# DanielPS555/Radix-sort-Merge-Sort-CUDA---Lab-y-practicos-GPGPU-2023

Hardware: AMD Instinct MI355X
Metric: Mkeys/s sorting uint32, n=2^28, 1 GPU (+ merge-sort at 2/4/8) (higher is better)
Workload: dtype u32; 1 GPU; LSD radix sort (8-bit digits, onesweep), n=2^28 uint32 u32, device-resident (BASELINE config 3); n_per_gpu=268435456, algo=radix, key=u32, dist=u32, parallelism=single GPU

## Files before the change

### include/labsort.h

```cpp
#ifndef LABSORT_H
#define LABSORT_H

#include <stddef.h>
#include <stdint.h>

#ifdef __cplusplus
extern "C" {
#endif

#define LABSORT_OK 0
#define LABSORT_ERR_ARG 1
#define LABSORT_ERR_HIP 2
#define LABSORT_ERR_DEVICE 3
#define LABSORT_ERR_PEER 4

#define LABSORT_ALGO_RADIX 0
#define LABSORT_ALGO_MERGE 1
#define LABSORT_ALGO_RADIX1 2
#define LABSORT_ALGO_AUTO 3
#define LABSORT_AUTO_MERGE_MAX_KEYS (1u << 16)
#define LABSORT_AUTO_PAIRS_MERGE_MAX_KEYS (1u << 18)

#define LABSORT_KEY_U32 0
#define LABSORT_KEY_I32 1
// ... 19 lines not shown
#define LABSORT_K_PARTITION 4
#define LABSORT_K_GSWEEP 5
#define LABSORT_K_GCOPY 6
#define LABSORT_K_COPY 7
#define LABSORT_K_MERGE4 8
#define LABSORT_K_SEGSORT 9
#define LABSORT_K_TOPK 10
#define LABSORT_K_COUNT 11

const char *labsort_version(void);
const char *labsort_error_string(int status);
int labsort_last_hip_error(void);
const char *labsort_hip_error_string(int hip_error);
size_t labsort_max_keys(int algo);
size_t labsort_tile_keys(void);
size_t labsort_merge_tile_keys(void);

size_t labsort_workspace_bytes(size_t n, int algo);
int labsort_sort_device(const void *d_in, void *d_out, size_t n, int key_type, int algo, void *d_workspace,
                        size_t workspace_bytes, void *stream);
int labsort_sort_host(void *h_keys, size_t n, int key_type, int algo);
int labsort_workspace_status(const void *d_workspace, size_t n, int algo, void *stream);
int labsort_radix_path(const void *d_workspace, size_t n, void *stream);
int labsort_pairs_workspace_status(const void *d_workspace, size_t n, int algo, void *stream);

#define LABSORT_XFER_AUTO 0
#define LABSORT_XFER_RCCL 1
#define LABSORT_XFER_PEER 2
#define LABSORT_MULTI_MAX_RANKS 8
#define LABSORT_MULTI_PHASES 9
#define LABSORT_MULTI_COLLECTIVES 3
int labsort_sort_host_multi(void *h_keys, size_t n, int key_type, int ngpus);
int labsort_sort_host_ranks(void *h_keys, size_t n, int key_type, int nranks, const int *devices, int transport);
int labsort_multi_timing(double *phase_ms, int nphases, size_t *max_sent_bytes);
int labsort_multi_collectives(double *arrive, double *leave, int nranks, int ncoll);
int labsort_multi_last_hip_error(void);
int labsort_multi_range_counts(size_t *counts, int nranks);
const char *labsort_multi_error_detail(void);
int labsort_multi_plan(const uint32_t *const *h_shards, const size_t *m, int nranks, int key_type, size_t *h_cuts);

#define LABSORT_COMM_ID_BYTES 128
#define LABSORT_DIST_MAX_RANKS 16
typedef struct labsort_comm *labsort_comm_t;
typedef struct {
    void *ctx;
    int (*allgather)(void *ctx, const void *h_in, void *h_out, size_t bytes);
// ... 84 lines not shown
```

### radix-sort-merge-sort-cuda---lab-y-practicos-gpgpu-2023_amd/__init__.py

```python
from __future__ import annotations

import ctypes
import os

import numpy as np

HERE = os.path.dirname(os.path.abspath(__file__))
LIB_PATH = os.environ.get("LABSORT_LIBRARY") or os.path.join(HERE, "liblabsort.so")

OK, ERR_ARG, ERR_HIP, ERR_DEVICE, ERR_PEER = 0, 1, 2, 3, 4
ALGO = {"radix": 0, "merge": 1, "radix1": 2, "auto": 3}
KEY = {"u32": 0, "i32": 1, "f32": 2, "bf16": 3, "f16": 4}
DIST = {"u32": 0, "u31": 1, "mod100": 2, "mod1000": 3, "sorted": 4, "reversed": 5, "const": 6, "lowbits": 7}
KCLASS = {"histogram": 0, "onesweep": 1, "tile_sort": 2, "merge": 3, "partition": 4, "gsweep": 5, "gcopy": 6,
          "copy": 7, "merge4": 8, "segsort": 9, "topk": 10}
TOPK_SORT_DIV = 4

C_SYMBOLS = [
    "labsort_version", "labsort_error_string", "labsort_last_hip_error", "labsort_hip_error_string",
    "labsort_max_keys", "labsort_tile_keys", "labsort_merge_tile_keys", "labsort_workspace_bytes",
    "labsort_sort_device", "labsort_sort_host", "labsort_wave_tile_sort", "labsort_tile_sort",
    "labsort_merge_parts", "labsort_merge_pass", "labsort_merge", "labsort_histogram", "labsort_fill",
    "labsort_count_descents", "labsort_timing_enable", "labsort_timing_read", "labsort_upper_bound", "sort",
    "labsort_merge_runs_workspace_bytes", "labsort_merge_runs",
    "labsort_pair_tile_keys", "labsort_pairs_workspace_bytes", "labsort_sort_pairs_device",
    "labsort_workspace_status", "labsort_pairs_workspace_status", "labsort_radix_path",
    "labsort_sort_host_multi", "labsort_sort_host_ranks", "labsort_multi_timing", "labsort_multi_last_hip_error",
    "labsort_multi_plan", "labsort_multi_error_detail", "labsort_multi_range_counts",
    "labsort_comm_unique_id", "labsort_comm_init_rccl", "labsort_comm_init_host", "labsort_comm_destroy",
    "labsort_dist_sort", "labsort_dist_timing", "labsort_dist_last_hip_error",
    "labsort_multi_collectives", "labsort_dist_collectives", "labsort_copy",
    "labsort_comm_set_timeout", "labsort_test_fault",
    "labsort_segment_tile_keys", "labsort_segment_pair_tile_keys", "labsort_segment_class_edges",
    "labsort_segments_workspace_bytes", "labsort_sort_segments_device", "labsort_sort_segments_pairs_device",
    "labsort_segments_workspace_status",
    "labsort_topk_workspace_bytes", "labsort_topk_device", "labsort_topk_workspace_status",
    "labsort_sort_rows_workspace_bytes", "labsort_sort_rows_device", "labsort_sort_rows_workspace_status",
    "labsort_sort16_chunk_keys", "labsort_sort16_workspace_bytes", "labsort_sort16_device",
    "labsort_sort16_workspace_status",
    "labsort_key_order_bits", "labsort_key_from_order_bits",
]
XFER = {"auto": 0, "rccl": 1, "peer": 2}
MULTI_PHASES = ["h2d", "local_sort", "plan", "exchange", "merge", "d2h", "total", "plan_work", "plan_wait"]
COLLECTIVES = ["samples", "counts", "grow"]
CXX_SYMBOLS = ["_Z11order_arrayPii", "_Z16order_with_trustPii"]


class LabsortError(RuntimeError):

# ... 55 lines not shown
    L.labsort_max_keys.argtypes = [i]
    L.labsort_tile_keys.restype = sz
    L.labsort_merge_tile_keys.restype = sz
    L.labsort_merge_parts.restype = sz
    L.labsort_merge_parts.argtypes = [sz]
    L.labsort_workspace_bytes.argtypes = [sz, i]
    L.labsort_sort_device.argtypes = [p, p, sz, i, i, p, sz, p]
    L.labsort_sort_host.argtypes = [p, sz, i, i]
    L.labsort_wave_tile_sort.argtypes = [p, sz, i, p]
    L.labsort_tile_sort.argtypes = [p, p, sz, i, p]
    L.labsort_merge_pass.argtypes = [p, p, sz, sz, i, p, p]
    L.labsort_merge.argtypes = [p, sz, p, sz, p, sz, sz, i, p, p]
    L.labsort_merge_runs_workspace_bytes.restype = sz
    L.labsort_merge_runs_workspace_bytes.argtypes = [sz]
    L.labsort_merge_runs.argtypes = [p, p, ctypes.POINTER(sz), i, i, p, sz, p]
    L.labsort_pair_tile_keys.restype = sz
    L.labsort_pair_tile_keys.argtypes = []
    L.labsort_pairs_workspace_bytes.restype = sz
    L.labsort_pairs_workspace_bytes.argtypes = [sz, i]
    L.labsort_sort_pairs_device.argtypes = [p, p, p, p, sz, i, i, p, sz, p]
    L.labsort_workspace_status.argtypes = [p, sz, i, p]
    if hasattr(L, "labsort_radix_path"):
        L.labsort_radix_path.argtypes = [p, sz, p]
    L.labsort_sort_host_multi.argtypes = [p, sz, i, i]
    L.labsort_sort_host_ranks.argtypes = [p, sz, i, i, p, i]
    L.labsort_multi_timing.argtypes = [ctypes.POINTER(ctypes.c_double), i, ctypes.POINTER(sz)]
    L.labsort_multi_plan.argtypes = [ctypes.POINTER(p), ctypes.POINTER(sz), i, i, ctypes.POINTER(sz)]
    L.labsort_multi_range_counts.argtypes = [ctypes.POINTER(sz), i]
    L.labsort_multi_error_detail.restype = ctypes.c_char_p
    L.labsort_multi_error_detail.argtypes = []
    L.labsort_comm_unique_id.argtypes = [p]
    L.labsort_comm_init_rccl.argtypes = [ctypes.POINTER(p), p, i, i]
    L.labsort_comm_init_host.argtypes = [ctypes.POINTER(p), i, i, ctypes.POINTER(HostColl)]
    L.labsort_comm_destroy.argtypes = [p]
    L.labsort_comm_set_timeout.argtypes = [p, ctypes.c_double]
    L.labsort_test_fault.argtypes = [ctypes.c_char_p, i]
    L.labsort_dist_sort.argtypes = [p, p, sz, i, p, ctypes.POINTER(p), ctypes.POINTER(sz), ctypes.POINTER(sz)]
    L.labsort_dist_timing.argtypes = [p, ctypes.POINTER(ctypes.c_double), i, ctypes.POINTER(sz)]
    L.labsort_dist_last_hip_error.argtypes = [p]
    L.labsort_multi_collectives.argtypes = [ctypes.POINTER(ctypes.c_double), ctypes.POINTER(ctypes.c_double), i, i]
    L.labsort_dist_collectives.argtypes = [p, ctypes.POINTER(ctypes.c_double), ctypes.POINTER(ctypes.c_double), i]
    L.labsort_copy.argtypes = [p, p, sz, p]
    L.labsort_pairs_workspace_status.argtypes = [p, sz, i, p]
    L.labsort_segment_tile_keys.restype = sz
    L.labsort_segment_tile_keys.argtypes = []
    L.labsort_segment_pair_tile_keys.restype = sz
# ... 284 lines not shown

def sort_device(d_in, d_out, n: int, key: str = "u32", algo: str = "radix", workspace=None,
                workspace_bytes_: int | None = None, stream=None) -> None:
    workspace, wsb, own = _workspace(workspace, lambda: workspace_bytes(n, algo))
    if workspace_bytes_ is not None:
        wsb = workspace_bytes_
    _check(lib.labsort_sort_device(_ptr(d_in), _ptr(d_out), n, KEY[key], ALGO[algo], _ptr(workspace), wsb,
                                   _stream(stream)), "sort_device")
    if own:
        workspace_status(workspace, n, algo, stream)


def workspace_status(workspace, n: int, algo: str = "radix", stream=None) -> None:
    _check(lib.labsort_workspace_status(_ptr(workspace), n, ALGO[algo], _stream(stream)), "sort_device (status)")


def radix_path(workspace, n: int, stream=None) -> int:
    r = int(lib.labsort_radix_path(_ptr(workspace), n, _stream(stream)))
    if r < 0:
        _check(-r, "radix_path")
    return r


def pairs_workspace_status(workspace, n: int, algo: str = "radix", stream=None) -> None:
    _check(lib.labsort_pairs_workspace_status(_ptr(workspace), n, ALGO[algo], _stream(stream)),
           "sort_pairs_device (status)")


def wave_tile_sort(d_keys, n: int, key: str = "u32", stream=None) -> None:
    _check(lib.labsort_wave_tile_sort(_ptr(d_keys), n, KEY[key], _stream(stream)), "wave_tile_sort")


def tile_sort(d_in, d_out, n: int, key: str = "u32", stream=None) -> None:
    _check(lib.labsort_tile_sort(_ptr(d_in), _ptr(d_out), n, KEY[key], _stream(stream)), "tile_sort")


def merge_pass(d_in, d_out, n: int, run: int, d_part, key: str = "u32", stream=None) -> None:
    _check(lib.labsort_merge_pass(_ptr(d_in), _ptr(d_out), n, run, KEY[key], _ptr(d_part), _stream(stream)),
           "merge_pass")


def merge(d_a, la: int, d_b, lb: int, d_out, d0: int, d1: int, d_part, key: str = "u32", stream=None) -> None:
    _check(lib.labsort_merge(_ptr(d_a) if la else 0, la, _ptr(d_b) if lb else 0, lb, _ptr(d_out), d0, d1,
                             KEY[key], _ptr(d_part), _stream(stream)), "merge")


# ... 224 lines not shown
```

### radix-sort-merge-sort-cuda---lab-y-practicos-gpgpu-2023_amd/csrc/api.hip

```cpp
#include <hip/hip_runtime.h>

#include <algorithm>
#include <cstdio>
#include <cstdlib>
#include <cstring>
#include <mutex>
#include <vector>

#include "host.h"
#include "segsort.h"

using namespace labsort;

namespace {

thread_local int g_last_hip = 0;

struct TimedLaunch {
    int cls;
    hipEvent_t a, b;
};
std::mutex g_timing_mu;
bool g_timing_on = false;
std::vector<TimedLaunch> g_pending;
// ... 92 lines not shown
    if (LABSORT_MERGE4)
        for (size_t r = (merge_levels(n, merge_tile(pairs)) % 2 ? 2 : 1) * merge_tile(pairs); r < n; r *= 4)
            bw = std::max(bw, merge4_bnd_words(n, r));
    L.off_bnd = c.take(bw * 4);
    for (int i = 0; i < 2; ++i) L.off_samp[i] = c.take(bw ? merge4_samp_words(n) * 4 : 0);
    L.total = c.o;
    return L;
}

bool use_gather(size_t n) {
    const char *e = std::getenv("LABSORT_RADIX_IMPL");
    if (e && !std::strcmp(e, "gather")) return true;
    if (n < GS_MIN_N || n >= GS_MAX_N) return false;
    return !(e && !std::strcmp(e, "onesweep"));
}

uint32_t hybrid_gate(size_t n) {
    const char *e = std::getenv("LABSORT_RADIX_HYBRID");
    if (e && !std::strcmp(e, "0")) return 0u;
    if (e && !std::strcmp(e, "2")) return HY_MAX_BUCKET;
    return n >= HY_MIN_N && n <= HY_MAX_N ? HY_FAST_GROUP : 0u;
}

bool small_path(size_t n, int algo) { return algo != LABSORT_ALGO_RADIX1 && n <= (size_t)TS_TILE; }

int sort_radix8(const uint32_t *ki, const uint32_t *vi, uint32_t *ko, uint32_t *vo, size_t n, uint32_t flip, char *ws,
                hipStream_t s) {
    const RadixLayout L = radix_layout(n, 8, OSP_TILE);
    Bufs b, vb;
    b.p[SEL_IN] = const_cast<uint32_t *>(ki);
    b.p[SEL_OUT] = ko;
    b.p[SEL_TMP] = reinterpret_cast<uint32_t *>(ws + L.off_tmp);
    vb.p[SEL_IN] = const_cast<uint32_t *>(vi);
    vb.p[SEL_OUT] = vo;
    vb.p[SEL_TMP] = vi ? reinterpret_cast<uint32_t *>(ws + align_up(L.total, 256)) : nullptr;
    uint32_t *hist = reinterpret_cast<uint32_t *>(ws + L.off_hist);
    uint32_t *counters = reinterpret_cast<uint32_t *>(ws + L.off_counter);
    uint32_t *err = reinterpret_cast<uint32_t *>(ws + L.off_err);
    uint32_t *lookback = reinterpret_cast<uint32_t *>(ws + L.off_lookback);
    Plan *plan = reinterpret_cast<Plan *>(ws + L.off_plan);
    HIP_TRY(launch_zero(ws, L.off_lookback, s));
    uint32_t *hps = reinterpret_cast<uint32_t *>(ws + L.off_hps);
    uint32_t *joint = reinterpret_cast<uint32_t *>(ws + L.off_joint);
    SegPlan *sps = reinterpret_cast<SegPlan *>(ws + L.off_segplan);
    const uint32_t hy_limit = vi ? 0u : hybrid_gate(n);
    const bool hyb = hy_limit != 0u;
    const HyCounts hc{reinterpret_cast<uint32_t *>(ws + L.off_hps2), reinterpret_cast<uint32_t *>(ws + L.off_top14), hy_limit};
    {
        TimingScope ts(LABSORT_K_HISTOGRAM, s);
        HIP_TRY(launch_hist_seg(ki, n, flip, hps, joint, s, hyb ? &hc : nullptr));
    }
    HIP_TRY(launch_plan8(hps, joint, n, ki == ko ? 1 : 0, plan, sps, hist, ws + L.off_lookback,
                         L.zero_bytes - L.off_lookback, s, hyb ? &hc : nullptr));
    for (int p = 0; p < L.P; ++p) {
        TimingScope ts(hyb && p < 2 ? LABSORT_K_UNTIMED : LABSORT_K_ONESWEEP, s);
        HIP_TRY(launch_onesweep_p(b, plan, p, n, flip, sps + p, lookback + (size_t)p * L.ntiles * L.R,
                                  counters + (size_t)p * OSP_NCTR, err, s, vi ? &vb : nullptr));
    }
    if (hyb) {
        TimingScope ts(LABSORT_K_SEGSORT, s);
        HIP_TRY(launch_hybrid_finish(plan, b, n, flip, hc.top14, reinterpret_cast<uint32_t *>(ws + L.off_fin_hdr),
                                     reinterpret_cast<uint32_t *>(ws + L.off_fin_off),
                                     reinterpret_cast<uint32_t *>(ws + L.off_fin_lists), s));
    }
    if (ki == ko) {
        HIP_TRY(launch_final_copy(b, plan, n, s));
        if (vi) HIP_TRY(launch_final_copy(vb, plan, n, s));
    }
    return LABSORT_OK;
}

int sort_radix1(const uint32_t *in, uint32_t *out, size_t n, uint32_t flip, char *ws, hipStream_t s) {
// ... 259 lines not shown
    }
    uint32_t err = 0;
    if (const int st = read_ws_words(d_ws, &err, 1, s)) return st;
    return err ? LABSORT_ERR_DEVICE : LABSORT_OK;
}
}

int labsort_workspace_status(const void *d_ws, size_t n, int algo, void *stream) {
    return read_status(d_ws, n != 0 && !small_path(n, resolve_algo(algo, n)), as_stream(stream));
}

int labsort_radix_path(const void *d_ws, size_t n, void *stream) {
    hipStream_t s = as_stream(stream);
    uint32_t hybrid = 0;
    hipError_t e = hipStreamSynchronize(s);
    const bool planned = n != 0 && d_ws && !small_path(n, LABSORT_ALGO_RADIX) && !use_gather(n) && n <= RADIX_MAX_N;
    if (e == hipSuccess && planned) {
        const size_t at = radix_layout(n, 8, OSP_TILE).off_plan + offsetof(Plan, hybrid);
        e = hipMemcpyAsync(&hybrid, static_cast<const char *>(d_ws) + at, 4, hipMemcpyDeviceToHost, s);
        if (e == hipSuccess) e = hipStreamSynchronize(s);
    }
    if (e != hipSuccess) return -fail_hip(e);
    return hybrid ? 1 : 0;
}

int labsort_pairs_workspace_status(const void *d_ws, size_t n, int algo, void *stream) {
    (void)algo;
    return read_status(d_ws, n > (size_t)TS_TILE_KV, as_stream(stream));
}

namespace {
bool host_pipe_enabled(size_t n, int algo) {
    if (algo == LABSORT_ALGO_RADIX1) return false;
    const char *e = std::getenv("LABSORT_HOST_PIPE");
    if (e && !std::strcmp(e, "0")) return false;
    return n >= (e && !std::strcmp(e, "1") ? (size_t)1 << 16 : HOST_PIPE_MIN);
}

int sort_host_pipelined(DeviceCache &c, void *h_keys, size_t n, int key_type, int algo) {
    const size_t m = (n + HOST_CHUNKS - 1) / HOST_CHUNKS;
    const int calgo = resolve_algo(algo, m);
    const size_t half = m * (HOST_CHUNKS / 2);
    int st;
    if ((st = ensure_buffer(&c.keys, &c.keys_bytes, n * 4))) return st;
    if ((st = ensure_buffer(&c.keys2, &c.keys2_bytes, n * 4))) return st;
    if ((st = ensure_buffer(&c.ws, &c.ws_bytes, labsort_workspace_bytes(m, calgo)))) return st;
// ... 308 lines not shown
```

### radix-sort-merge-sort-cuda---lab-y-practicos-gpgpu-2023_amd/csrc/common.h

```cpp
#pragma once
#include <hip/hip_runtime.h>
#include <stddef.h>
#include <stdint.h>

namespace labsort {

constexpr int WAVE = 64;

__host__ __device__ inline uint32_t f32_ord(uint32_t x) {
    if ((x & 0x7FFFFFFFu) > 0x7F800000u) return 0xFFFFFFFFu;
    return (x & 0x80000000u) ? ~x : x | 0x80000000u;
}
__host__ __device__ inline uint32_t f32_unord(uint32_t o) { return (o & 0x80000000u) ? o & 0x7FFFFFFFu : ~o; }

constexpr uint32_t BF16_NAN_T = 0x7F80u, F16_NAN_T = 0x7C00u;
__host__ __device__ inline uint32_t ord16(uint32_t x, uint32_t nan_t) {
    x &= 0xFFFFu;
    if ((x & 0x7FFFu) > nan_t) return 0xFFFFu;
    return (x & 0x8000u) ? ~x & 0xFFFFu : x | 0x8000u;
}
__host__ __device__ inline uint32_t unord16(uint32_t o) { return (o & 0x8000u) ? o & 0x7FFFu : ~o & 0xFFFFu; }

constexpr int RADIX_BITS = 8;
constexpr int OS_BLOCK = 512;
// ... 69 lines not shown
constexpr uint32_t NEXT_NONE = 0xFFFFFFFFu;

struct Plan {
    uint32_t src[MAX_PASSES];
    uint32_t dst[MAX_PASSES];
    uint32_t next[MAX_PASSES];
    uint32_t prev[MAX_PASSES];
    uint32_t copy_from;
    uint32_t active;
    uint32_t hybrid;
    uint32_t fin_src;
};

constexpr int HY_TOP_BITS = 14, HY_TOP = 1 << HY_TOP_BITS;
constexpr uint32_t HY_BUCKETS = 1u << 16;
constexpr uint32_t HY_MAX_BUCKET = 32768;
constexpr size_t HY_MIN_N = ((size_t)1 << 28) - ((size_t)1 << 24);
constexpr size_t HY_MAX_N = ((size_t)1 << 28) + 3 * ((size_t)1 << 24);
constexpr uint32_t HY_FAST_GROUP = 4u * 5120u;
struct HyCounts {
    uint32_t *hps2;
    uint32_t *top14;
    uint32_t limit;
};

struct Bufs {
    uint32_t *p[3];
};

constexpr uint32_t LB_AGG = 1u << 30;
constexpr uint32_t LB_INC = 2u << 30;
constexpr uint32_t LB_VAL = (1u << 30) - 1u;
constexpr size_t RADIX_MAX_N = (size_t)LB_VAL;

hipError_t launch_fill(uint32_t *out, size_t n, uint64_t seed, int dist, uint64_t param, uint64_t first,
                       hipStream_t s);
hipError_t launch_histogram(const uint32_t *keys, size_t n, uint32_t flip, int bits, uint32_t *hist,
                            hipStream_t s);
hipError_t launch_plan(const uint32_t *hist, size_t n, int bits, int in_is_out, Plan *plan, hipStream_t s);
hipError_t launch_onesweep(Bufs b, const Plan *plan, int pass, int bits, size_t n, uint32_t flip,
                           const uint32_t *hist, uint32_t *lookback, uint32_t *counter, uint32_t *err,
                           hipStream_t s);
hipError_t launch_hist_seg(const uint32_t *keys, size_t n, uint32_t flip, uint32_t *hps, uint32_t *joint,
                           hipStream_t s, const HyCounts *hy = nullptr);
hipError_t launch_plan8(const uint32_t *hps, const uint32_t *joint, size_t n, int in_is_out, Plan *plan,
                        SegPlan *segplans, uint32_t *hist, void *zero_p, size_t zero_bytes, hipStream_t s,
                        const HyCounts *hy = nullptr);
hipError_t launch_onesweep_p(Bufs b, const Plan *plan, int pass, size_t n, uint32_t flip, const SegPlan *sp,
                             uint32_t *lookback, uint32_t *counter, uint32_t *err, hipStream_t s,
                             const Bufs *vb = nullptr);
hipError_t launch_final_copy(Bufs b, const Plan *plan, size_t n, hipStream_t s);
hipError_t launch_tile_sort(const uint32_t *in, uint32_t *out, size_t n, uint32_t flip, hipStream_t s,
                            uint32_t *samp_out = nullptr);
hipError_t launch_wave_tile_sort(uint32_t *keys, size_t n, uint32_t flip, hipStream_t s);
hipError_t launch_merge_pass(const uint32_t *in, uint32_t *out, size_t n, size_t run, uint32_t flip,
                             hipStream_t s, const uint32_t *vin = nullptr, uint32_t *vout = nullptr,
                             const MgPairs *pairs = nullptr, uint32_t *samp_out = nullptr);
hipError_t launch_tile_sort_kv(const uint32_t *in, uint32_t *out, const uint32_t *vin, uint32_t *vout, size_t n,
                               uint32_t flip, hipStream_t s, uint32_t *samp_out = nullptr);
#ifndef LABSORT_M4_S
#define LABSORT_M4_S 128
#endif
constexpr uint32_t M4_S = LABSORT_M4_S;
inline size_t merge4_samp_words(size_t n) { return (n + M4_S - 1) / M4_S + 4; }
size_t merge4_bnd_words(size_t n, size_t r);
hipError_t launch_merge4_pass(const uint32_t *in, uint32_t *out, size_t n, size_t r, uint32_t flip, uint32_t *bnd,
                              const uint32_t *samp_in, uint32_t *samp_out, hipStream_t s, const uint32_t *vin = nullptr,
// ... 19 lines not shown
```

### radix-sort-merge-sort-cuda---lab-y-practicos-gpgpu-2023_amd/csrc/kernels.hip

```cpp
#include "common.h"
#include "devutil.h"
#include "host.h"
#include "lds_pass.h"

#include <cstdlib>
#include <cstring>
#include <type_traits>

namespace labsort {

__device__ __forceinline__ uint64_t mix64(uint64_t z) {
    z += 0x9E3779B97F4A7C15ull;
    z = (z ^ (z >> 30)) * 0xBF58476D1CE4E5B9ull;
    z = (z ^ (z >> 27)) * 0x94D049BB133111EBull;
    return z ^ (z >> 31);
}

__global__ __launch_bounds__(256) void k_fill(uint32_t *__restrict__ out, size_t n, uint64_t seed, int dist,
                                              uint64_t param, uint64_t first) {
    const size_t stride = (size_t)gridDim.x * blockDim.x;
    for (size_t i = (size_t)blockIdx.x * blockDim.x + threadIdx.x; i < n; i += stride) {
        const uint64_t gi = first + i;
        const uint64_t z = mix64(seed ^ (gi * 0x9E3779B97F4A7C15ull));
        const uint32_t hi = (uint32_t)(z >> 32);
// ... 87 lines not shown
    __syncthreads();
    if (threadIdx.x != 0) return;
    int act[MAX_PASSES];
    int k = 0;
    for (int p = 0; p < MAX_PASSES; ++p) {
        plan->src[p] = SEL_SKIP;
        plan->dst[p] = SEL_SKIP;
        if (p < P && !triv[p]) act[k++] = p;
    }
    plan->active = (uint32_t)k;
    plan_buffers(plan, act, k, in_is_out);
}

template <bool HY>
__global__ __launch_bounds__(HIST_BLOCK) void k_hist_seg(const uint32_t *__restrict__ keys, size_t n, uint32_t flip,
                                                         uint32_t *__restrict__ hps, uint32_t *__restrict__ joint,
                                                         uint32_t bps, HyCounts hy) {
    constexpr int SL = 32;
    constexpr int JF = 4096;
    constexpr int NJ = HY ? 2 : 3;
    __shared__ uint32_t h[256 * SL];
    __shared__ uint32_t hj[NJ * JF];
    __shared__ uint32_t ht[HY ? HY_TOP : 1];
    for (int i = threadIdx.x; i < 256 * SL; i += HIST_BLOCK) h[i] = 0u;
    for (int i = threadIdx.x; i < NJ * JF; i += HIST_BLOCK) hj[i] = 0u;
    if constexpr (HY) {
        for (int i = threadIdx.x; i < HY_TOP; i += HIST_BLOCK) ht[i] = 0u;
    }
    __syncthreads();
    const uint32_t slot = threadIdx.x & (SL - 1);
    auto count = [&](uint32_t k) {
        k ^= flip;
        atomicAdd(&h[(k & 255u) * SL + slot], 1u);
#pragma unroll
        for (int p = 0; p < NJ; ++p) atomicAdd(&hj[p * JF + ((k >> (8 * p + 4)) & (JF - 1))], 1u);
        if constexpr (HY) atomicAdd(&ht[k >> (32 - HY_TOP_BITS)], 1u);
    };
    auto fld = [&](uint32_t k, int p) { return (k >> (8 * p + 4)) & (JF - 1); };
    auto count16 = [&](const uint4 (&c)[4]) {
        uint32_t k[16];
#pragma unroll
        for (int u = 0; u < 4; ++u) {
            k[4 * u] = c[u].x ^ flip;
            k[4 * u + 1] = c[u].y ^ flip;
            k[4 * u + 2] = c[u].z ^ flip;
            k[4 * u + 3] = c[u].w ^ flip;
// ... 170 lines not shown
__global__ __launch_bounds__(256) void k_plan8(const uint32_t *__restrict__ hps, const uint32_t *__restrict__ joint,
                                               uint32_t n, int in_is_out, int seg_later, Plan *__restrict__ plan,
                                               SegPlan *__restrict__ sps, uint32_t *__restrict__ hist_out,
                                               uint4 *__restrict__ zp, size_t zn4, HyCounts hy) {
    constexpr uint32_t PW = 4;
    if (blockIdx.x >= PW) {
        const size_t stride = (size_t)(gridDim.x - PW) * blockDim.x;
        for (size_t i = (size_t)(blockIdx.x - PW) * blockDim.x + threadIdx.x; i < zn4; i += stride)
            zp[i] = make_uint4(0u, 0u, 0u, 0u);
        return;
    }
    const int me = (int)blockIdx.x;
    __shared__ uint32_t hist[4 * 256];
    __shared__ uint32_t sh[NSEG * 256 + 8];
    __shared__ uint32_t triv[4];
    __shared__ uint32_t start[NSEG + 1];
    __shared__ uint32_t prevs[4];
    __shared__ int first;
    __shared__ uint32_t max14;
    const uint32_t t = threadIdx.x;
    if (t < 4) triv[t] = 0;
    if (t == 0) max14 = 0u;
    __syncthreads();
    if (hy.top14) {
        uint32_t m = 0;
        for (uint32_t i = t; i < (uint32_t)HY_TOP; i += 256u) m = max(m, hy.top14[i]);
        atomicMax(&max14, m);
    }
    uint32_t v[4] = {0, 0, 0, 0};
    for (int s = 0; s < NSEG; ++s) {
        v[0] += hps[s * 256 + t];
#pragma unroll
        for (int p = 1; p < 4; ++p) v[p] += joint[(p * NSEG + s) * 256 + t];
    }
#pragma unroll
    for (int p = 0; p < 4; ++p) {
        hist[p * 256 + t] = v[p];
        if (me == 0) hist_out[p * 256 + t] = v[p];
        if (v[p] == n) triv[p] = 1;
    }
    if (t <= (uint32_t)NSEG) start[t] = seg_later < 0 ? (t ? n : 0u) : seg_start(t, n);
    __syncthreads();
    const bool hybrid = hy.top14 && !triv[0] && !triv[1] && max14 <= min(hy.limit, HY_MAX_BUCKET);
    __syncthreads();
    if (hybrid && t < 2) triv[t] = 1;
    __syncthreads();
    if (t == 0 && me != 0) {
        int k = 0, last = -1;
        for (int p = 0; p < 4; ++p) {
            prevs[p] = NEXT_NONE;
            if (!triv[p]) {
                if (last >= 0) prevs[p] = (uint32_t)last;
                last = p;
                if (!k++) first = p;
            }
        }
        if (!k) first = -1;
    }
    if (t == 0 && me == 0) {
        int act[4];
        int k = 0;
        for (int p = 0; p < MAX_PASSES; ++p) {
            plan->src[p] = SEL_SKIP;
            plan->dst[p] = SEL_SKIP;
            plan->next[p] = NEXT_NONE;
            plan->prev[p] = NEXT_NONE;
// ... 1075 lines not shown
    const unsigned g = (unsigned)((n + OS_TILE - 1) / OS_TILE);
    k_onesweep<1, OS_BLOCK, OS_KPT><<<g, OS_BLOCK, 0, s>>>(b, plan, pass, (uint32_t)n, flip, hist, lookback, counter,
                                                           err);
    return hipGetLastError();
}

hipError_t launch_onesweep_p(Bufs b, const Plan *plan, int pass, size_t n, uint32_t flip, const SegPlan *sp,
                             uint32_t *lookback, uint32_t *counter, uint32_t *err, hipStream_t s, const Bufs *vb) {
    if (n > RADIX_MAX_N) return hipErrorInvalidValue;
    const size_t ntiles = (n + OSP_TILE - 1) / OSP_TILE + NSEG;
    const size_t want = (size_t)cu_count();
    const unsigned g = (unsigned)(ntiles < want ? ntiles : want);
    if (vb)
        k_onesweep_p<true><<<g, OSP_KV_BLOCK, 0, s>>>(b, plan, pass, (uint32_t)n, flip, sp, lookback, counter, err, *vb);
    else
        k_onesweep_p<false><<<g, OSP_BLOCK, 0, s>>>(b, plan, pass, (uint32_t)n, flip, sp, lookback, counter, err, b);
    return hipGetLastError();
}


hipError_t launch_hist_seg(const uint32_t *keys, size_t n, uint32_t flip, uint32_t *hps, uint32_t *joint,
                           hipStream_t s, const HyCounts *hy) {
    if (n == 0) return hipSuccess;
    size_t bps = n / ((size_t)NSEG * HS_MIN_KEYS);
    bps = bps < 1 ? 1 : bps > (size_t)HS_BPS ? (size_t)HS_BPS : bps;
    if (hy) k_hist_seg<true><<<NSEG * (unsigned)bps, HIST_BLOCK, 0, s>>>(keys, n, flip, hps, joint, (uint32_t)bps, *hy);
    else k_hist_seg<false><<<NSEG * (unsigned)bps, HIST_BLOCK, 0, s>>>(keys, n, flip, hps, joint, (uint32_t)bps, HyCounts{});
    return hipGetLastError();
}

hipError_t launch_plan8(const uint32_t *hps, const uint32_t *joint, size_t n, int in_is_out, Plan *plan,
                        SegPlan *segplans, uint32_t *hist, void *zero_p, size_t zero_bytes, hipStream_t s,
                        const HyCounts *hy) {
    const bool fold = zero_bytes % 16 == 0;
    if (!fold && zero_bytes) {
        const hipError_t z = launch_zero(zero_p, zero_bytes, s);
        if (z != hipSuccess) return z;
    }
    const size_t zn4 = fold ? zero_bytes / 16 : 0;
    const unsigned g = 4u + (zn4 ? blocks_for(zn4, 256 * 4, 2048) : 0u);
    k_plan8<<<g, 256, 0, s>>>(hps, joint, (uint32_t)n, in_is_out, 1, plan, segplans, hist,
                              static_cast<uint4 *>(zero_p), zn4, hy ? *hy : HyCounts{});
    return hipGetLastError();
}


__global__ __launch_bounds__(256) void k_zero(uint4 *__restrict__ p4, size_t n4, uint32_t *__restrict__ tail,
                                             uint32_t ntail) {
// ... 120 lines not shown
```

Baseline: 141,700 Mkeys/s.

## Add lean hybrid histogram pass that predicts hybrid path and skips full histogram

Adds a lean histogram kernel that first samples keys to predict whether the hybrid radix path will be taken. If so, it counts only digit 2 and the top-14-bit buckets, decides the verdict in the last block, and fills the joint histogram so the full hist_seg kernel can return early. The aim is to cut the per-key counting work in the first histogram pass for inputs that go hybrid. The cost is an extra kernel launch, and a misprediction means the full histogram still runs after the lean one.

```diff
diff --git a/harness/lean_predict_check.py b/harness/lean_predict_check.py
--- /dev/null
+++ b/harness/lean_predict_check.py
@@ -0,0 +1,42 @@
+import numpy as np
+M=np.uint64
+def mix64(z):
+    z = z + M(0x9E3779B97F4A7C15)
+    z = (z ^ (z >> M(30))) * M(0xBF58476D1CE4E5B9)
+    z = (z ^ (z >> M(27))) * M(0x94D049BB133111EB)
+    return z ^ (z >> M(31))
+def gen(pos, seed, dist, n):
+    gi = pos.astype(np.uint64)
+    z = mix64(M(seed) ^ (gi * M(0x9E3779B97F4A7C15)))
+    hi = (z >> M(32)).astype(np.uint32)
+    if dist=="u32": return hi
+    if dist=="u31": return (z >> M(33)).astype(np.uint32)
+    if dist=="mod1000": return hi % np.uint32(1000)
+    if dist=="sorted": return gi.astype(np.uint32)
+def positions(n):
+    r = np.arange(256, dtype=np.uint64)
+    span = n // 256
+    room = span - 63
+    off = ((r * M(2654435761)) & M(0xFFFFFFFF)) >> M(8)
+    start = r * M(span) + off % M(room)
+    return (start[:,None] + np.arange(64,dtype=np.uint64)[None,:]).ravel()
+def predict(keys, n, limit):
+    a = np.bitwise_and.reduce(keys); o = np.bitwise_or.reduce(keys); d = int(a ^ o)
+    bins = np.bincount(keys >> np.uint32(28), minlength=16)
+    maxc = int(bins.max())
+    thr = 5*limit*16384*1024/(4*n)
+    likely = (d & 255)!=0 and ((d>>8)&255)!=0 and maxc*n*4 <= 5*limit*16384*1024
+    return likely, maxc, thr
+LIM=20480
+with np.errstate(over='ignore'):
+    for n,dist in [(15<<24,"u32"),(1<<28,"u32"),(19<<24,"u32"),(1<<28,"u31"),(1<<28,"sorted"),(1<<28,"mod1000")]:
+        for seed in (0x5EED0003, 1, 2, 3):
+            k = gen(positions(n), seed, dist, n)
+            l, maxc, thr = predict(k, n, LIM)
+            print(f"n={n/(1<<24):5.1f}x2^24 {dist:8s} seed={seed:#x} likely={l} max bin {maxc} threshold {thr:.1f}")
+    rng = np.random.default_rng(1)
+    mx = np.array([np.bincount(rng.integers(0,16,16384),minlength=16).max() for _ in range(20000)])
+    thr = 5*LIM*16384*1024/(4*(19<<24))
+    print("u32, 20000 samples: largest bin mean %.1f max %d; threshold at 19x2^24 %.1f (bin sd %.1f -> %.1f sd above the mean bin 1024)" % (mx.mean(), mx.max(), thr, (16384*15/256)**.5, (thr-1024)/(16384*15/256)**.5))
+    mn = np.array([np.bincount(rng.integers(0,8,16384),minlength=8).max() for _ in range(20000)])
+    print("u31 at 2^28: largest bin min %d, threshold %.1f" % (mn.min(), 5*LIM*16384*1024/(4*(1<<28))))
diff --git a/include/labsort.h b/include/labsort.h
--- a/include/labsort.h
+++ b/include/labsort.h
@@ -65,6 +65,7 @@
 int labsort_sort_host(void *h_keys, size_t n, int key_type, int algo);
 int labsort_workspace_status(const void *d_workspace, size_t n, int algo, void *stream);
 int labsort_radix_path(const void *d_workspace, size_t n, void *stream);
+int labsort_radix_counting(const void *d_workspace, size_t n, void *stream);
 int labsort_pairs_workspace_status(const void *d_workspace, size_t n, int algo, void *stream);
 
 #define LABSORT_XFER_AUTO 0
diff --git a/radix-sort-merge-sort-cuda---lab-y-practicos-gpgpu-2023_amd/__init__.py b/radix-sort-merge-sort-cuda---lab-y-practicos-gpgpu-2023_amd/__init__.py
--- a/radix-sort-merge-sort-cuda---lab-y-practicos-gpgpu-2023_amd/__init__.py
+++ b/radix-sort-merge-sort-cuda---lab-y-practicos-gpgpu-2023_amd/__init__.py
@@ -25,6 +25,7 @@
     "labsort_merge_runs_workspace_bytes", "labsort_merge_runs",
     "labsort_pair_tile_keys", "labsort_pairs_workspace_bytes", "labsort_sort_pairs_device",
     "labsort_workspace_status", "labsort_pairs_workspace_status", "labsort_radix_path",
+    "labsort_radix_counting",
     "labsort_sort_host_multi", "labsort_sort_host_ranks", "labsort_multi_timing", "labsort_multi_last_hip_error",
     "labsort_multi_plan", "labsort_multi_error_detail", "labsort_multi_range_counts",
     "labsort_comm_unique_id", "labsort_comm_init_rccl", "labsort_comm_init_host", "labsort_comm_destroy",
@@ -126,6 +127,8 @@
     L.labsort_workspace_status.argtypes = [p, sz, i, p]
     if hasattr(L, "labsort_radix_path"):
         L.labsort_radix_path.argtypes = [p, sz, p]
+    if hasattr(L, "labsort_radix_counting"):
+        L.labsort_radix_counting.argtypes = [p, sz, p]
     L.labsort_sort_host_multi.argtypes = [p, sz, i, i]
     L.labsort_sort_host_ranks.argtypes = [p, sz, i, i, p, i]
     L.labsort_multi_timing.argtypes = [ctypes.POINTER(ctypes.c_double), i, ctypes.POINTER(sz)]
@@ -456,6 +459,13 @@
     return r
 
 
+def radix_counting(workspace, n: int, stream=None) -> int:
+    r = int(lib.labsort_radix_counting(_ptr(workspace), n, _stream(stream)))
+    if r < 0:
+        _check(-r, "radix_counting")
+    return r
+
+
 def pairs_workspace_status(workspace, n: int, algo: str = "radix", stream=None) -> None:
     _check(lib.labsort_pairs_workspace_status(_ptr(workspace), n, ALGO[algo], _stream(stream)),
            "sort_pairs_device (status)")
diff --git a/radix-sort-merge-sort-cuda---lab-y-practicos-gpgpu-2023_amd/csrc/api.hip b/radix-sort-merge-sort-cuda---lab-y-practicos-gpgpu-2023_amd/csrc/api.hip
--- a/radix-sort-merge-sort-cuda---lab-y-practicos-gpgpu-2023_amd/csrc/api.hip
+++ b/radix-sort-merge-sort-cuda---lab-y-practicos-gpgpu-2023_amd/csrc/api.hip
@@ -138,6 +138,13 @@
     return n >= HY_MIN_N && n <= HY_MAX_N ? HY_FAST_GROUP : 0u;
 }
 
+uint32_t hy_count_mode() {
+    const char *e = std::getenv("LABSORT_HY_COUNT");
+    if (e && !std::strcmp(e, "lean")) return HY_COUNT_LEAN;
+    if (e && !std::strcmp(e, "full")) return HY_COUNT_FULL;
+    return HY_COUNT_AUTO;
+}
+
 bool small_path(size_t n, int algo) { return algo != LABSORT_ALGO_RADIX1 && n <= (size_t)TS_TILE; }
 
 int sort_radix8(const uint32_t *ki, const uint32_t *vi, uint32_t *ko, uint32_t *vo, size_t n, uint32_t flip, char *ws,
@@ -161,9 +168,11 @@
     SegPlan *sps = reinterpret_cast<SegPlan *>(ws + L.off_segplan);
     const uint32_t hy_limit = vi ? 0u : hybrid_gate(n);
     const bool hyb = hy_limit != 0u;
-    const HyCounts hc{reinterpret_cast<uint32_t *>(ws + L.off_hps2), reinterpret_cast<uint32_t *>(ws + L.off_top14), hy_limit};
+    const HyCounts hc{reinterpret_cast<uint32_t *>(ws + L.off_hps2), reinterpret_cast<uint32_t *>(ws + L.off_top14), hy_limit,
+                      err, hy_count_mode()};
     {
         TimingScope ts(LABSORT_K_HISTOGRAM, s);
+        if (hyb) HIP_TRY(launch_hist_lean(ki, n, flip, joint, s, hc));
         HIP_TRY(launch_hist_seg(ki, n, flip, hps, joint, s, hyb ? &hc : nullptr));
     }
     HIP_TRY(launch_plan8(hps, joint, n, ki == ko ? 1 : 0, plan, sps, hist, ws + L.off_lookback,
@@ -469,6 +478,21 @@
     }
     if (e != hipSuccess) return -fail_hip(e);
     return hybrid ? 1 : 0;
+}
+
+int labsort_radix_counting(const void *d_ws, size_t n, void *stream) {
+    hipStream_t s = as_stream(stream);
+    uint32_t ran[2] = {0, 0};
+    if (n == 0 || !d_ws || small_path(n, LABSORT_ALGO_RADIX) || use_gather(n) || n > RADIX_MAX_N) return 0;
+    hipError_t e = hipStreamSynchronize(s);
+    if (e == hipSuccess) {
+        static_assert(HY_CTL_FULL == HY_CTL_LEAN + 1, "read together");
+        const size_t at = radix_layout(n, 8, OSP_TILE).off_err + HY_CTL_LEAN * 4;
+        e = hipMemcpyAsync(ran, static_cast<const char *>(d_ws) + at, 8, hipMemcpyDeviceToHost, s);
+        if (e == hipSuccess) e = hipStreamSynchronize(s);
+    }
+    if (e != hipSuccess) return -fail_hip(e);
+    return ran[0] ? (ran[1] ? 2 : 1) : 0;
 }
 
 int labsort_pairs_workspace_status(const void *d_ws, size_t n, int algo, void *stream) {
diff --git a/radix-sort-merge-sort-cuda---lab-y-practicos-gpgpu-2023_amd/csrc/common.h b/radix-sort-merge-sort-cuda---lab-y-practicos-gpgpu-2023_amd/csrc/common.h
--- a/radix-sort-merge-sort-cuda---lab-y-practicos-gpgpu-2023_amd/csrc/common.h
+++ b/radix-sort-merge-sort-cuda---lab-y-practicos-gpgpu-2023_amd/csrc/common.h
@@ -115,7 +115,25 @@
     uint32_t *hps2;
     uint32_t *top14;
     uint32_t limit;
+    uint32_t *ctl;
+    uint32_t mode;
 };
+constexpr uint32_t HY_CTL_TICKET = 1;
+constexpr uint32_t HY_CTL_NAND = 2;
+constexpr uint32_t HY_CTL_OR = 3;
+constexpr uint32_t HY_CTL_VERDICT = 4;
+constexpr uint32_t HY_CTL_LEAN = 5;
+constexpr uint32_t HY_CTL_FULL = 6;
+constexpr uint32_t HY_VERDICT_CLASSIC = 1, HY_VERDICT_HYBRID = 2;
+constexpr uint32_t HY_COUNT_AUTO = 0, HY_COUNT_LEAN = 1, HY_COUNT_FULL = 2;
+#ifndef LABSORT_HY_LEAN_SL
+#define LABSORT_HY_LEAN_SL 32
+#endif
+constexpr int HY_LEAN_SL = LABSORT_HY_LEAN_SL;
+inline uint32_t hist_seg_bps(size_t n) {
+    const size_t bps = n / ((size_t)NSEG * HS_MIN_KEYS);
+    return (uint32_t)(bps < 1 ? 1 : bps > (size_t)HS_BPS ? (size_t)HS_BPS : bps);
+}
 
 struct Bufs {
     uint32_t *p[3];
@@ -136,6 +154,8 @@
                            hipStream_t s);
 hipError_t launch_hist_seg(const uint32_t *keys, size_t n, uint32_t flip, uint32_t *hps, uint32_t *joint,
                            hipStream_t s, const HyCounts *hy = nullptr);
+hipError_t launch_hist_lean(const uint32_t *keys, size_t n, uint32_t flip, uint32_t *joint, hipStream_t s,
+                            const HyCounts &hy);
 hipError_t launch_plan8(const uint32_t *hps, const uint32_t *joint, size_t n, int in_is_out, Plan *plan,
                         SegPlan *segplans, uint32_t *hist, void *zero_p, size_t zero_bytes, hipStream_t s,
                         const HyCounts *hy = nullptr);
diff --git a/radix-sort-merge-sort-cuda---lab-y-practicos-gpgpu-2023_amd/csrc/hist_lean.hip b/radix-sort-merge-sort-cuda---lab-y-practicos-gpgpu-2023_amd/csrc/hist_lean.hip
--- /dev/null
+++ b/radix-sort-merge-sort-cuda---lab-y-practicos-gpgpu-2023_amd/csrc/hist_lean.hip
@@ -0,0 +1,253 @@
+#include "common.h"
+#include "devutil.h"
+
+namespace labsort {
+
+namespace {
+
+constexpr uint32_t HY_SAMPLE_RUNS = 256, HY_SAMPLE_RUN = 64, HY_SAMPLE = HY_SAMPLE_RUNS * HY_SAMPLE_RUN;
+constexpr uint32_t HY_COARSE_BITS = 4, HY_COARSE = 1u << HY_COARSE_BITS;
+static_assert(HY_SAMPLE == 16 * HIST_BLOCK, "16 sample keys per thread, one run per wave and round");
+
+__device__ bool predict_hybrid(const uint32_t *__restrict__ keys, size_t n, uint32_t flip, uint32_t limit, uint32_t *sc) {
+    const uint32_t t = threadIdx.x, lane = t & 63u, wid = t >> 6;
+    uint32_t *sand = sc + 32 * HY_COARSE, *sor = sand + 1;
+    if (t < 32 * HY_COARSE) sc[t] = 0u;
+    if (t == 0) {
+        *sand = ~0u;
+        *sor = 0u;
+    }
+    __syncthreads();
+    const size_t span = n / HY_SAMPLE_RUNS;
+    const uint32_t room = (uint32_t)(span - (HY_SAMPLE_RUN - 1));
+    uint32_t x[16];
+#pragma unroll
+    for (uint32_t j = 0; j < 16u; ++j) {
+        const uint32_t r = j * 16u + wid;
+        const size_t pos = (size_t)r * span + ((r * 2654435761u) >> 8) % room + lane;
+        x[j] = keys[pos];
+    }
+    uint32_t a = ~0u, o = 0u;
+#pragma unroll
+    for (uint32_t j = 0; j < 16u; ++j) {
+        const uint32_t k = x[j] ^ flip;
+        a &= k;
+        o |= k;
+        atomicAdd(&sc[(k >> (32 - HY_COARSE_BITS)) * 32u + (lane & 31u)], 1u);
+    }
+    wave_and_or(a, o);
+    if (lane == 0) {
+        atomicAnd(sand, a);
+        atomicOr(sor, o);
+    }
+    __syncthreads();
+    uint32_t c = 0;
+    if (t < 64u) {
+#pragma unroll
+        for (uint32_t q = 0; q < 8u; ++q) c += sc[(t >> 2) * 32u + (t & 3u) * 8u + q];
+        c += __shfl_xor(c, 1);
+        c += __shfl_xor(c, 2);
+#pragma unroll
+        for (int off = 4; off < 64; off <<= 1) c = max(c, (uint32_t)__shfl_xor(c, off));
+    }
+    const uint32_t diff = *sand ^ *sor;
+    __syncthreads();
+    if (t == 0) sc[0] = c;
+    __syncthreads();
+    const uint32_t maxc = sc[0];
+    __syncthreads();
+    if ((diff & 255u) == 0u || ((diff >> 8) & 255u) == 0u) return false;
+    const uint64_t groups = HY_TOP >> HY_COARSE_BITS;
+    return (uint64_t)maxc * n * 4u <= (uint64_t)5u * limit * HY_SAMPLE * groups;
+}
+
+}
+
+template <int SL>
+__global__ __launch_bounds__(HIST_BLOCK) void k_hist_lean(const uint32_t *__restrict__ keys, size_t n, uint32_t flip,
+                                                          uint32_t *__restrict__ joint, uint32_t bps, HyCounts hy) {
+    static_assert(256 * SL >= 32 * (int)HY_COARSE + 2, "the sample's counters fit the digit-2 counters");
+    __shared__ uint32_t h2[256 * SL];
+    __shared__ uint32_t ht[HY_TOP];
+    __shared__ uint32_t red[4];
+    const uint32_t t = threadIdx.x, lane = t & 63u;
+    if (hy.mode == HY_COUNT_FULL) return;
+    if (hy.mode != HY_COUNT_LEAN && !predict_hybrid(keys, n, flip, hy.limit, h2)) return;
+    if (blockIdx.x == 0 && t == 0) hy.ctl[HY_CTL_LEAN] = 1u;
+    for (int i = t; i < 256 * SL; i += HIST_BLOCK) h2[i] = 0u;
+    for (int i = t; i < HY_TOP; i += HIST_BLOCK) ht[i] = 0u;
+    if (t == 0) {
+        red[0] = ~0u;
+        red[1] = 0u;
+        red[2] = 0u;
+    }
+    __syncthreads();
+    constexpr int NU = 4;
+    const uint32_t slot = t & (SL - 1);
+    uint32_t ka = ~0u, ko = 0u;
+    auto dig2 = [&](uint32_t k) { return (k >> 16) & 255u; };
+    auto top = [&](uint32_t k) { return k >> (32 - HY_TOP_BITS); };
+    auto count = [&](uint32_t k) {
+        k ^= flip;
+        ka &= k;
+        ko |= k;
+        atomicAdd(&h2[dig2(k) * SL + slot], 1u);
+        atomicAdd(&ht[top(k)], 1u);
+    };
+    auto count16 = [&](const uint4 (&c)[4]) {
+        uint32_t k[16];
+#pragma unroll
+        for (int u = 0; u < 4; ++u) {
+            k[4 * u] = c[u].x ^ flip;
+            k[4 * u + 1] = c[u].y ^ flip;
+            k[4 * u + 2] = c[u].z ^ flip;
+            k[4 * u + 3] = c[u].w ^ flip;
+        }
+#pragma unroll
+        for (int j = 0; j < 16; ++j) {
+            ka &= k[j];
+            ko |= k[j];
+        }
+        if (__ballot(top(k[0]) == top(k[3])) == 0ull) {
+#pragma unroll
+            for (int j = 0; j < 16; ++j) atomicAdd(&h2[dig2(k[j]) * SL + slot], 1u);
+#pragma unroll
+            for (int j = 0; j < 16; ++j) atomicAdd(&ht[top(k[j])], 1u);
+            return;
+        }
+        auto add_field = [&](auto &&fv, auto &&ctr) {
+            const uint32_t f0 = fv(k[0]);
+            bool same = fv(k[15]) == f0;
+            if (same) {
+#pragma unroll
+                for (int j = 1; j < 15; ++j) same &= fv(k[j]) == f0;
+            }
+            const uint32_t w0 = __builtin_amdgcn_readfirstlane(f0);
+            const uint64_t act = __ballot(true);
+            if (__ballot(same && f0 == w0) == act) {
+                if (mbcnt64(act) == 0u) atomicAdd(ctr(w0), 16u * (uint32_t)__popcll(act));
+                return;
+            }
+            if (same) {
+                atomicAdd(ctr(f0), 16u);
+                return;
+            }
+#pragma unroll
+            for (int u = 0; u < 4; ++u) {
+                const uint32_t fa = fv(k[4 * u]);
+                const bool s4 = fv(k[4 * u + 3]) == fa && fv(k[4 * u + 1]) == fa && fv(k[4 * u + 2]) == fa;
+                if (s4) {
+                    atomicAdd(ctr(fa), 4u);
+                } else {
+#pragma unroll
+                    for (int j = 4 * u; j < 4 * u + 4; ++j) atomicAdd(ctr(fv(k[j])), 1u);
+                }
+            }
+        };
+        add_field(dig2, [&](uint32_t f) { return &h2[f * SL + slot]; });
+        add_field(top, [&](uint32_t f) { return &ht[f]; });
+    };
+    const uint32_t seg = blockIdx.x / bps, part = blockIdx.x % bps;
+    const size_t sb = seg_start(seg, n), se = seg_start(seg + 1, n);
+    const size_t per = (se - sb + bps - 1) / bps;
+    const size_t beg = sb + (size_t)part * per < se ? sb + (size_t)part * per : se;
+    const size_t end = beg + per < se ? beg + per : se;
+    if ((((uintptr_t)keys) & 15u) == 0) {
+        const size_t abeg = (beg + 3) & ~(size_t)3;
+        const size_t vbeg = abeg < end ? abeg : end;
+        for (size_t i = beg + t; i < vbeg; i += HIST_BLOCK) count(keys[i]);
+        const size_t nv = (end - vbeg) / 4;
+        const uint4 *v = reinterpret_cast<const uint4 *>(keys + vbeg);
+        size_t i = t;
+        uint4 c[NU], x[NU];
+        if (i + (NU - 1) * HIST_BLOCK < nv) {
+#pragma unroll
+            for (int u = 0; u < NU; ++u) c[u] = ld_stream4<NT_HIST>(v + i + u * HIST_BLOCK);
+        }
+        for (; i + (NU - 1) * HIST_BLOCK < nv; i += NU * HIST_BLOCK) {
+            if (i + (2 * NU - 1) * HIST_BLOCK < nv) {
+#pragma unroll
+                for (int u = 0; u < NU; ++u) x[u] = ld_stream4<NT_HIST>(v + i + (NU + u) * HIST_BLOCK);
+            }
+            count16(c);
+#pragma unroll
+            for (int u = 0; u < NU; ++u) c[u] = x[u];
+        }
+        for (; i < nv; i += HIST_BLOCK) {
+            const uint4 y = ld_stream4<NT_HIST>(v + i);
+            count(y.x); count(y.y); count(y.z); count(y.w);
+        }
+        for (size_t r = vbeg + nv * 4 + t; r < end; r += HIST_BLOCK) count(keys[r]);
+    } else {
+        for (size_t i = beg + t; i < end; i += HIST_BLOCK) count(keys[i]);
+    }
+    wave_and_or(ka, ko);
+    if (lane == 0) {
+        atomicAnd(&red[0], ka);
+        atomicOr(&red[1], ko);
+    }
+    __syncthreads();
+    if (t < 256u) {
+        uint32_t c = 0;
+#pragma unroll 8
+        for (int q = 0; q < SL; ++q) c += h2[t * SL + ((q + t) & (SL - 1))];
+        if (c) atomicAdd(&hy.hps2[seg * 256 + t], c);
+    }
+    const uint32_t rot = (blockIdx.x * 1088u) & (uint32_t)(HY_TOP - 1);
+    for (uint32_t i0 = t; i0 < (uint32_t)HY_TOP; i0 += HIST_BLOCK) {
+        const uint32_t i = (i0 + rot) & (uint32_t)(HY_TOP - 1);
+        const uint32_t c = ht[i];
+        if (c) atomicAdd(&hy.top14[i], c);
+    }
+    if (t == 0) {
+        atomicOr(&hy.ctl[HY_CTL_NAND], ~red[0]);
+        atomicOr(&hy.ctl[HY_CTL_OR], red[1]);
+    }
+    __threadfence();
+    __syncthreads();
+    if (t == 0) red[3] = atomicAdd(&hy.ctl[HY_CTL_TICKET], 1u) == gridDim.x - 1u ? 1u : 0u;
+    __syncthreads();
+    if (red[3] == 0u) return;
+    __threadfence();
+    uint32_t s4[4], m = 0;
+#pragma unroll
+    for (uint32_t q = 0; q < 4u; ++q) {
+        s4[q] = 0;
+#pragma unroll
+        for (uint32_t j = 0; j < 4u; ++j) {
+            const uint32_t c = ld_agent(&hy.top14[16u * t + 4u * q + j]);
+            s4[q] += c;
+            m = max(m, c);
+        }
+    }
+#pragma unroll
+    for (int off = 32; off > 0; off >>= 1) m = max(m, (uint32_t)__shfl_xor(m, off));
+    if (lane == 0) atomicMax(&red[2], m);
+    __syncthreads();
+    const uint32_t diff = ~ld_agent(&hy.ctl[HY_CTL_NAND]) ^ ld_agent(&hy.ctl[HY_CTL_OR]);
+    const bool hybrid = (diff & 255u) != 0u && ((diff >> 8) & 255u) != 0u && red[2] <= min(hy.limit, HY_MAX_BUCKET);
+    if (t == 0) hy.ctl[HY_CTL_VERDICT] = hybrid ? HY_VERDICT_HYBRID : HY_VERDICT_CLASSIC;
+    if (!hybrid) return;
+#pragma unroll
+    for (uint32_t q = 0; q < 4u; ++q) {
+        const uint32_t f = 4u * t + q;
+        joint[(3u * NSEG + (f & 15u)) * 256 + (f >> 4)] = s4[q];
+    }
+    if (t < 256u) {
+        uint32_t tot = 0;
+        for (int s = 0; s < NSEG; ++s) tot += ld_agent(&hy.hps2[s * 256 + t]);
+        joint[(2u * NSEG) * 256 + t] = tot;
+    }
+}
+
+hipError_t launch_hist_lean(const uint32_t *keys, size_t n, uint32_t flip, uint32_t *joint, hipStream_t s,
+                            const HyCounts &hy) {
+    if (n == 0) return hipSuccess;
+    HyCounts h = hy;
+    if (n < HY_SAMPLE && h.mode == HY_COUNT_AUTO) h.mode = HY_COUNT_LEAN;
+    const uint32_t bps = hist_seg_bps(n);
+    k_hist_lean<HY_LEAN_SL><<<NSEG * bps, HIST_BLOCK, 0, s>>>(keys, n, flip, joint, bps, h);
+    return hipGetLastError();
+}
+
+}
diff --git a/radix-sort-merge-sort-cuda---lab-y-practicos-gpgpu-2023_amd/csrc/kernels.hip b/radix-sort-merge-sort-cuda---lab-y-practicos-gpgpu-2023_amd/csrc/kernels.hip
--- a/radix-sort-merge-sort-cuda---lab-y-practicos-gpgpu-2023_amd/csrc/kernels.hip
+++ b/radix-sort-merge-sort-cuda---lab-y-practicos-gpgpu-2023_amd/csrc/kernels.hip
@@ -133,6 +133,12 @@
     __shared__ uint32_t h[256 * SL];
     __shared__ uint32_t hj[NJ * JF];
     __shared__ uint32_t ht[HY ? HY_TOP : 1];
+    if constexpr (HY) {
+        if (hy.ctl) {
+            if (hy.ctl[HY_CTL_VERDICT] == HY_VERDICT_HYBRID) return;
+            if (blockIdx.x == 0 && threadIdx.x == 0) hy.ctl[HY_CTL_FULL] = 1u;
+        }
+    }
     for (int i = threadIdx.x; i < 256 * SL; i += HIST_BLOCK) h[i] = 0u;
     for (int i = threadIdx.x; i < NJ * JF; i += HIST_BLOCK) hj[i] = 0u;
     if constexpr (HY) {
@@ -349,7 +355,8 @@
     if (t < 4) triv[t] = 0;
     if (t == 0) max14 = 0u;
     __syncthreads();
-    if (hy.top14) {
+    const uint32_t verdict = hy.ctl ? hy.ctl[HY_CTL_VERDICT] : 0u;
+    if (hy.top14 && verdict == 0u) {
         uint32_t m = 0;
         for (uint32_t i = t; i < (uint32_t)HY_TOP; i += 256u) m = max(m, hy.top14[i]);
         atomicMax(&max14, m);
@@ -368,7 +375,8 @@
     }
     if (t <= (uint32_t)NSEG) start[t] = seg_later < 0 ? (t ? n : 0u) : seg_start(t, n);
     __syncthreads();
-    const bool hybrid = hy.top14 && !triv[0] && !triv[1] && max14 <= min(hy.limit, HY_MAX_BUCKET);
+    const bool hybrid = verdict ? verdict == HY_VERDICT_HYBRID
+                                : hy.top14 && !triv[0] && !triv[1] && max14 <= min(hy.limit, HY_MAX_BUCKET);
     __syncthreads();
     if (hybrid && t < 2) triv[t] = 1;
     __syncthreads();
@@ -1490,8 +1498,7 @@
 hipError_t launch_hist_seg(const uint32_t *keys, size_t n, uint32_t flip, uint32_t *hps, uint32_t *joint,
                            hipStream_t s, const HyCounts *hy) {
     if (n == 0) return hipSuccess;
-    size_t bps = n / ((size_t)NSEG * HS_MIN_KEYS);
-    bps = bps < 1 ? 1 : bps > (size_t)HS_BPS ? (size_t)HS_BPS : bps;
+    const uint32_t bps = hist_seg_bps(n);
     if (hy) k_hist_seg<true><<<NSEG * (unsigned)bps, HIST_BLOCK, 0, s>>>(keys, n, flip, hps, joint, (uint32_t)bps, *hy);
     else k_hist_seg<false><<<NSEG * (unsigned)bps, HIST_BLOCK, 0, s>>>(keys, n, flip, hps, joint, (uint32_t)bps, HyCounts{});
     return hipGetLastError();
```

Result: faster. 146,100 Mkeys/s, median of 6 (+3.1%).
